# pr0g/ToyMeshPathTracer

Measured on AMD Instinct MI355X. Metric: MRays/s on sponza.obj 1920x1080 64spp at 1/2/4/8 GPUs; %HBM roofline, higher is better.
Workload: dtype f32

## Files before the change

### toymeshpathtracer_amd/csrc/tmpt_api.cpp

```cpp
#include <dlfcn.h>
#include <hip/hip_runtime.h>
#include <rccl/rccl.h>
#include <string.h>

#include <algorithm>
#include <new>
#include <chrono>
#include <string>
#include <thread>
#include <vector>

#include "tmpt.h"
#include "tmpt_internal.h"
#include "tmpt_traverse.h"
#include "tmpt_render.h"

namespace tmpt {

static thread_local std::string g_last_error;
void set_error(const std::string& msg) { g_last_error = msg; }
const char* last_error() { return g_last_error.c_str(); }

int load_obj(const char* path, std::vector<float>& tris, f3& bmin, f3& bmax);
void camera_init(tmpt_camera* cam, f3 lookFrom, f3 lookAt, f3 vup, float vfov, float aspect,
// ... 69 lines not shown
    {"builder", true, 0, 1, &Options::builder, nullptr, nullptr},
    {"layout", true, 0, 1, &Options::layout, nullptr, nullptr},
    {"leaf_max", true, 1, kLeafMaxTris, &Options::leaf_max, nullptr, nullptr},
    {"collapse", true, 0, 1, &Options::collapse, nullptr, nullptr},
    {"ploc_radius", true, 1, 256, &Options::ploc_radius, nullptr, nullptr},
    {"sah_c_leaf", true, 0, 1e6, nullptr, &Options::sah_c_leaf, nullptr},
    {"sah_c_tri", true, 0, 1e6, nullptr, &Options::sah_c_tri, nullptr},
    {"sample_block", false, 0, 1024, &Options::sample_block, nullptr, nullptr},
    {"sample_tail", false, -1, 64, &Options::sample_tail, nullptr, nullptr},
    {"sbuf_max", false, 0, 1e18, nullptr, nullptr, &Options::sbuf_max},
    {"sbuf_pair", false, 0, 1, &Options::sbuf_pair, nullptr, nullptr},
    {"pilot", false, -1, 512, &Options::pilot, nullptr, nullptr},
    {"help", false, -1, 1, &Options::help, nullptr, nullptr},
    {"pair", false, -1, 63, &Options::pair, nullptr, nullptr},
    {"balance", false, 0, 1, &Options::balance, nullptr, nullptr},
    {"dprio", false, 0, 1, &Options::dprio, nullptr, nullptr},
    {"wave_cap", false, 0, 64, &Options::wave_cap, nullptr, nullptr},
    {"pixel_chains", false, -1, 1024, &Options::pixel_chains, nullptr, nullptr},
    {"tie_defer", false, -1, 1, &Options::tie_defer, nullptr, nullptr},
    {"redo_cap", false, 0, 1 << 30, &Options::redo_cap, nullptr, nullptr},
    {"redo_inline", false, 0, 1, &Options::redo_inline, nullptr, nullptr},
    {"redo_lanes", false, 1, 64, &Options::redo_lanes, nullptr, nullptr},
    {"path_waves", false, 0, 5, &Options::path_waves, nullptr, nullptr},
    {"rowspec", false, 0, 1, &Options::rowspec, nullptr, nullptr},
    {"rowspec_wmax", false, 0, 16384, &Options::rowspec_wmax, nullptr, nullptr},
    {"rowspec_windows", false, 0, 32, &Options::rowspec_windows, nullptr, nullptr},
    {"rowspec_spread", false, -1, 100, nullptr, &Options::rowspec_spread, nullptr},
    {"rowspec_groups", false, 1, kRowSpecMaxGroups, &Options::rowspec_groups, nullptr, nullptr},
    {"rowspec_noshadow", false, 0, 1, &Options::rowspec_noshadow, nullptr, nullptr},
    {"rowspec_chase", false, 0, 1, &Options::rowspec_chase, nullptr, nullptr},
    {"rowspec_stream", false, 0, 1, &Options::rowspec_stream, nullptr, nullptr},
    {"rowstream_dynamic", false, 0, 1, &Options::rowstream_dynamic, nullptr, nullptr},
    {"row_flag_leaves", false, 0, 1, &Options::row_flag_leaves, nullptr, nullptr},
    {"row_occ", false, 0, 5, &Options::row_occ, nullptr, nullptr},
    {"wf_bins", false, 1, 8, &Options::wf_bins, nullptr, nullptr},
    {"rowstream_test_abort", false, 0, 1, &Options::rowstream_test_abort, nullptr, nullptr},
    {"tie_rule", false, 0, 1, &Options::tie_rule, nullptr, nullptr},
    {"aov_group", false, 0, 16, &Options::aov_group, nullptr, nullptr},
};

const OptionDef* find_option(const char* key)
{
    for (const OptionDef& d : kOptions)
        if (strcmp(d.name, key) == 0) return &d;
    return nullptr;
}
// ... 812 lines not shown
```

### toymeshpathtracer_amd/csrc/tmpt_internal.h

```cpp
#pragma once

#include <hip/hip_runtime.h>
#include <stdint.h>

#include <string>
#include <vector>

#include "tmpt_math.h"

namespace tmpt {

struct alignas(16) Bvh4Node {
    float4 a;
    uint4 b;
    uint4 c;
    int4 d;
};
static_assert(sizeof(Bvh4Node) == 64, "BVH4Q node is one half cache line");

constexpr int kLeafCountShift = 27;
constexpr uint32_t kLeafFirstMask = (1u << kLeafCountShift) - 1u;
constexpr int kLeafMaxTris = 16;
constexpr int kTopNodes = 120;
constexpr int kTopNodes5 = 80;
// ... 45 lines not shown
};

void build_octree(const float* tris9, int32_t n, const float bmin[3], const float bmax[3], OctreeHost& out);
uint64_t octree_digest(const OctreeHost& t);
void octree_grid(const OctreeHost& t, const float bmin[3], const float bmax[3], OctGrid& g);
int32_t octree_flat_triangles(const float* tris9, int32_t n, const OctGrid& g, std::vector<uint8_t>& flat);

struct SoaScene {
    const uint4* __restrict__ na = nullptr;
    const uint4* __restrict__ nb = nullptr;
    const uint2* __restrict__ nc = nullptr;
    const int4* __restrict__ nd = nullptr;
    const float4* __restrict__ ta = nullptr;
    const float4* __restrict__ tb = nullptr;
    const float2* __restrict__ tc = nullptr;
};

constexpr float kBoxPadRel = 1e-5f;
constexpr float kTfarSlack = 1.00001f;

constexpr int kStackTotal = 128;

constexpr int kRowSpecMaxGroups = 8;
constexpr int kRenderCounters = 32;
constexpr int kTieCounter = 24;
constexpr int kCrackCounter = 30;
constexpr int kRedoRaysCounter = 31;
constexpr int kRedoCounter = 26;

struct Options {
    int builder = 0;
    int layout = 0;
    int leaf_max = 2;
    int collapse = 0;
    int ploc_radius = 32;
    float sah_c_leaf = 0.7f, sah_c_tri = 0.5f;
    int sample_block = 0;
    int rowstream_dynamic = 1;
    int row_flag_leaves = 1;
    int row_occ = 0;
    int sample_tail = -1;
    double sbuf_max = 0.0;
    int sbuf_pair = 1;
    int pilot = -1;
    int help = -1;
    int pair = -1;
    int balance = 1;
    int dprio = 1;
    int wave_cap = 0;
    int pixel_chains = -1;
    int rowspec = 1;
    int rowspec_wmax = 0;
    int rowspec_windows = 0;
    float rowspec_spread = -1.0f;
    int rowspec_groups = 2;
    int rowspec_noshadow = 1;
    int rowspec_chase = 1;
    int rowspec_stream = 1;
    int rowstream_test_abort = 0;
    int wf_bins = 1;
    int tie_rule = 0;
    int tie_defer = -1;
    int redo_cap = 0;
    int redo_lanes = 4;
    int path_waves = 0;
    int redo_inline = 1;
    int aov_group = 0;
};
int options_parse(Options& o, const char* text, bool allow_build);
int options_set(Options& o, const char* key, double value, bool allow_build);
int options_get(const Options& o, const char* key, double* value);

struct Scene {
    int device = 0;
    int32_t n = 0;
    int32_t n_nodes = 0;
    int32_t max_depth = 0;
    Bvh4Node* nodes4 = nullptr;
    int32_t n_nodes4 = 0, depth4 = 0, leaf_max = 0, ploc_iters = 0;
    TriPre* tri_pre = nullptr;
    TriOrig* tri_orig = nullptr;
    void* soa_buf = nullptr;
    SoaScene soa;
    std::vector<float> tris_host;
    OctNode* oct = nullptr;
    int32_t* oct_refs = nullptr;
    OctView* oct_view = nullptr;
    int32_t n_oct = 0, oct_leaves = 0, oct_depth = 0;
    int32_t oct_flat = 0;
// ... 85 lines not shown
```

### toymeshpathtracer_amd/csrc/tmpt_render.hip

```cpp
#include <hip/hip_runtime.h>

#include <stdio.h>
#include <stdlib.h>
#include <string.h>

#include <algorithm>
#include <chrono>
#include <cmath>
#include <vector>

#include "tmpt_render.h"

namespace tmpt {

__device__ __forceinline__ uint64_t wballot(bool p) { return __builtin_amdgcn_ballot_w64(p); }
__device__ __forceinline__ bool wany(bool p) { return __builtin_amdgcn_ballot_w64(p) != 0; }

__device__ __forceinline__ uint64_t stamp()
{
    uint64_t t;
    __builtin_amdgcn_sched_barrier(0);
    asm volatile("s_memtime %0\n\ts_waitcnt lgkmcnt(0)" : "=s"(t)::"memory");
    __builtin_amdgcn_sched_barrier(0);
    return t;
// ... 725 lines not shown
    const uint32_t* __restrict__ dprio_cost;
    uint32_t lane_cap;
    uint32_t chunk;
    uint32_t nblk, blk;
    uint32_t blk0;
    uint32_t ua;
    float4* __restrict__ sbuf;
    uint32_t sb_ss, sb_sp;
    uint32_t pair;
    const uint32_t* __restrict__ upix;
    const uint32_t* __restrict__ ustate;
    float4* __restrict__ rs_out;
    uint32_t* __restrict__ rs_end;
    const uint32_t* __restrict__ p_dev;
    int rs_noshadow;
    const uint32_t* __restrict__ uslot;
    RsStream rss;
    uint2* __restrict__ redo;
    float4* __restrict__ redo_state;
    uint32_t redo_cap;
    uint32_t redo_inline;
    uint32_t redo_lanes;
    uint32_t oct_shadow;
};

constexpr uint32_t kSimdKeys = 8u * 8u * 2u * 16u * 4u;

__device__ __forceinline__ uint2 simd_rank(uint32_t* reg)
{
    uint32_t r = 0, d = 0;
    if (lane_id() == 0) {
        const uint32_t hw = (uint32_t)__builtin_amdgcn_s_getreg((31 << 11) | 4);
        const uint32_t xcc = (uint32_t)__builtin_amdgcn_s_getreg((31 << 11) | 20) & 7u;
        const uint32_t key = ((((xcc * 8u + ((hw >> 13) & 7u)) * 2u + ((hw >> 12) & 1u)) * 16u +
                               ((hw >> 8) & 15u)) * 4u) + ((hw >> 4) & 3u);
        r = hw & 15u;
        if (atomicAdd(&reg[2 * key], 1u) == 0) {
            d = atomicAdd(&reg[2 * kSimdKeys], 1u);
            __hip_atomic_store(&reg[2 * key + 1], d + 1u, __ATOMIC_RELAXED, __HIP_MEMORY_SCOPE_AGENT);
        } else {
            uint32_t v;
            while ((v = __hip_atomic_load(&reg[2 * key + 1], __ATOMIC_RELAXED, __HIP_MEMORY_SCOPE_AGENT)) == 0u)
                __builtin_amdgcn_s_sleep(2);
            d = v - 1u;
        }
    }
// ... 211 lines not shown
                atomicAdd(&counters[21], 1ull);
            }
        } else if (lane_id() == 0) {
            atomicAdd(&counters[20 + (rd.x >= pc.wps ? 2 : 3)], 1ull);
        }
        if (res >= res_end)
            for (int k = 0; k < 6; ++k) __builtin_amdgcn_s_sleep(127);
    }
#ifdef TMPT_EXP_WAVETIME
    const int wt_id = (int)(gtid >> 6);
    if (lane_id() == 0 && wt_id < kWaveTimeMax) g_wavetime[3 * wt_id] = __builtin_amdgcn_s_memrealtime();
#endif
    bool has_pix = false, in_query = false, qany = false;
    bool helper = false, waiting = false;
    uint32_t hown = 0;
    uint32_t pix = 0, rng = 0, smp = 0, depth = 0;
    uint32_t pf0 = 0, pf1 = 0, pf2 = 0, pf3 = 0, pf_smp = 0xFFFFFFFFu, pf_pix = 0;
    uint32_t cur_unit = 0, re0 = 0, rs0 = 0, ndraw = 0;
    bool single = false;
    uint32_t psteps = 0;
    uint64_t rs_nr = 0, rs_nl = 0, rs_lr = 0, rs_ll = 0, rs_sr = 0, rs_sl = 0, rs_st = 0;
    uint64_t pt_shade = 0, pt_node = 0, pt_leaf = 0, pt_t = PROF ? stamp() : 0;
    uint64_t ps_fetch = 0, ps_shade = 0, ps_cam = 0, ps_start = 0;
    f3 col = mk(0.0f, 0.0f, 0.0f);
    TravRay r;
    TravState ts;
    trav_init(ts, kMaxT);

    for (;;) {
        const bool wants = has_pix ? !in_query : (HELP && helper ? !in_query : !exhausted);
        const uint64_t need = wballot(wants);
        const uint64_t trav = wballot(in_query);
        int shade_min = SHADE_MIN;
        if (TAIL > 0) {
            const int act = __popcll(wballot(has_pix));
            shade_min = max(1, min(SHADE_MIN, act / TAIL));
        }
        if (need != 0 && (__popcll(need) >= shade_min || trav == 0)) {
            if (COUNT || PROF >= 3) {
                ++rs_sr;
                rs_sl += (uint64_t)__popcll(need);
                rs_st += (uint64_t)__popcll(trav);
            }
            bool cam = false, start = false, sany = false;
            f3 so = mk(0.0f, 0.0f, 0.0f), sd = so;
            const uint64_t nopix = wballot(!has_pix && !(HELP && helper) && !exhausted);
// ... 375 lines not shown
                    camera_sample(a.cam, (uint32_t)x, y, a.invW, a.invH, rng, so, sd, ndraw);
                } else {
                    camera_sample(a.cam, (uint32_t)x, y, a.invW, a.invH, rng, so, sd);
                }
                start = true;
            }
            if (PROF >= 2) {
                const uint64_t t = stamp();
                ps_cam += t - ps_t;
                ps_t = t;
            }
            if (start) {
                r = make_trav_ray(so, sd);
                trav_init(ts, kMaxT);
                qany = sany;
                if (sany) ++rays_s; else ++rays_e;
                in_query = sv.n > 0 && !ray_has_nan(so, sd);
                if (!DEFER && a.root_check && cam && in_query && !octree_root_hit(sv, so, sd, kMinT, kMaxT)) {
                    in_query = false;
                    atomicAdd(&sv.oct->ties[1], 1ull);
                }
            }
            if (PROF >= 2) ps_start += stamp() - ps_t;
        }
        if (dp0 > 0.0f) {
            float rem = 0.0f;
            if (has_pix)
                rem = smp > (uint32_t)a.smp_begin
                          ? (float)psteps * (float)((uint32_t)a.smp_end - smp) *
                                __builtin_amdgcn_rcpf((float)(smp - (uint32_t)a.smp_begin))
                          : 3.0e38f;
            for (int o = 32; o > 0; o >>= 1) rem = fmaxf(rem, __shfl_xor(rem, o));
            if (rem >= dp0) __builtin_amdgcn_s_setprio(3);
            else if (rem >= dp1) __builtin_amdgcn_s_setprio(2);
            else if (rem >= dp2) __builtin_amdgcn_s_setprio(1);
            else __builtin_amdgcn_s_setprio(0);
        }
        if (PROF) {
            const uint64_t t = stamp();
            pt_shade += t - pt_t;
            pt_t = t;
        }
        if (!wany(in_query)) {
            if (exhausted && !wany(has_pix)) break;
            if (SAMP == 4 && !wany(has_pix)) {
                const uint32_t tick = rss_ld32(&pc.rss.ctl[2]);
// ... 2 lines not shown
                    wd_tick = tick;
                    wd_time = now;
                } else if (now - wd_time > (uint64_t)pc.rss.watchdog) {
                    if (lane_id() == 0) atomicExch(&pc.rss.ctl[1], 1u);
                    exhausted = true;
                }
                __builtin_amdgcn_s_sleep(32);
            }
            continue;
        }
        for (int k = 0; k < STEPS; ++k) {
            const uint64_t q = wballot(in_query);
            const uint64_t at_leaf = q & wballot(ts.node < 0);
            const uint64_t at_node = q & ~at_leaf;
            if (q == 0) break;
            const uint32_t n_leaf = (uint32_t)__builtin_popcount((uint32_t)at_leaf) +
                                    (uint32_t)__builtin_popcount((uint32_t)(at_leaf >> 32));
            const uint32_t n_node = (uint32_t)__builtin_popcount((uint32_t)at_node) +
                                    (uint32_t)__builtin_popcount((uint32_t)(at_node >> 32));
            const bool leaf_round = n_leaf > n_node;
            if (COUNT || PROF >= 3) {
                if (!leaf_round) { ++rs_nr; rs_nl += (uint64_t)__popcll(at_node); }
                if (leaf_round) { ++rs_lr; rs_ll += (uint64_t)__popcll(at_leaf); }
            }
            if (!COUNT) {
                const bool stepping = in_query && ((ts.node < 0) == leaf_round);
                bool done = false;
                if (leaf_round) {
                    if (stepping) done = trav_step4q2_mixed<false, BLOCK, SL, true, 2, SOA, false, FLAG>(sv, r, qany, ts, st, cnt);
                } else {
                    if (stepping) done = trav_step4q2_mixed<false, BLOCK, SL, true, 1, SOA, false, FLAG>(sv, r, qany, ts, st, cnt);
                }
                if (done) in_query = false;
                if (stepping && ((kFull && pc.cost_out) || dp0 > 0.0f)) ++psteps;
            } else if (in_query && (ts.node < 0) == leaf_round) {
                TravCount c1;
                if (trav_step4q2_mixed<COUNT, BLOCK, SL, true, 0, SOA, false, FLAG>(sv, r, qany, ts, st, c1)) in_query = false;
                TravCount& dst = qany ? cnt_s : cnt;
                dst.nodes += c1.nodes;
                dst.tris += c1.tris;
                if ((kFull && pc.cost_out) || dp0 > 0.0f) ++psteps;
            }
            if (PROF) {
                const uint64_t t = stamp();
                (leaf_round ? pt_leaf : pt_node) += t - pt_t;
                pt_t = t;
            }
        }
    }
#ifdef TMPT_EXP_WAVETIME
    if (lane_id() == 0 && wt_id < kWaveTimeMax) g_wavetime[3 * wt_id + 1] = __builtin_amdgcn_s_memrealtime();
#endif
    if (DEFER && pc.redo_inline) {
        constexpr uint64_t kRedoGuard = 2000000;
        const unsigned long long waves = (unsigned long long)gridDim.x * (BLOCK / 64);
        uint32_t t = 0;
        if (lane_id() == 0) {
            atomicAdd(&counters[kRedoWaves], 1ull);
            t = (uint32_t)atomicAdd(&counters[kRedoTaken], (unsigned long long)pc.redo_lanes);
        }
        t = lane_id() < pc.redo_lanes ? (uint32_t)__shfl((int)t, 0) + lane_id() : 0xFFFFFFFFu;
        unsigned long long seen = ~0ull;
        uint64_t since = 0;
        for (;;) {
            const unsigned long long listed =
                __hip_atomic_load(&counters[kRedoCounter], __ATOMIC_RELAXED, __HIP_MEMORY_SCOPE_AGENT);
            const uint32_t lim = (uint32_t)min(listed, (unsigned long long)pc.redo_cap);
            uint2 e = make_uint2(kRedoEmpty, 0u);
// ... 46 lines not shown
            atomicAdd(&counters[2], (unsigned long long)nt);
            atomicAdd(&counters[4], (unsigned long long)nvs);
            atomicAdd(&counters[5], (unsigned long long)nts);
        }
        if (COUNT || PROF >= 3) {
            atomicAdd(&counters[6], (unsigned long long)rs_nr);
            atomicAdd(&counters[7], (unsigned long long)rs_nl);
            atomicAdd(&counters[8], (unsigned long long)rs_lr);
            atomicAdd(&counters[9], (unsigned long long)rs_ll);
            atomicAdd(&counters[10], (unsigned long long)rs_sr);
            atomicAdd(&counters[11], (unsigned long long)rs_sl);
            atomicAdd(&counters[12], (unsigned long long)rs_st);
        }
        if (PROF) {
            atomicAdd(&counters[13], (unsigned long long)pt_shade);
            atomicAdd(&counters[14], (unsigned long long)pt_node);
            atomicAdd(&counters[15], (unsigned long long)pt_leaf);
        }
        if (PROF >= 2) {
            atomicAdd(&counters[16], (unsigned long long)ps_fetch);
            atomicAdd(&counters[17], (unsigned long long)ps_shade);
            atomicAdd(&counters[18], (unsigned long long)ps_cam);
            atomicAdd(&counters[19], (unsigned long long)ps_start);
        }
    }
}

__global__ void __launch_bounds__(256) k_pair_order(const uint32_t* __restrict__ order, int64_t P, int32_t h,
                                                     uint32_t* __restrict__ paired)
{
    const int64_t r = (int64_t)blockIdx.x * 256 + threadIdx.x;
    if (r >= P) return;
    const int64_t full = P / 64, c = r / 64, i = r - c * 64;
    const int64_t m = c < full ? 64 : P - full * 64;
    const int64_t hc = c < full ? h : (m * h + 63) / 64;
    const int64_t src = i < hc ? c * h + i : P - 1 - (c * (64 - h) + (i - hc));
    paired[r] = order[src];
}

__global__ void __launch_bounds__(256) k_order_keys(const uint32_t* __restrict__ cost, int32_t W,
                                                     int32_t rows, uint32_t* __restrict__ keys,
                                                     uint32_t* __restrict__ vals)
{
    const int64_t i = (int64_t)blockIdx.x * 256 + threadIdx.x;
    if (i >= (int64_t)W * rows) return;
    const int y = (int)(i / W), x = (int)(i - (int64_t)y * W);
// ... 631 lines not shown
struct PixelChains {
    const uint32_t* cpix;
    const float4* cinit;
    int n, smp0, cspp;
};
int render_rowspec(Scene& s, const RenderArgs& a, uint32_t* d_out, unsigned long long* d_counters,
                   const PixelChains* ch = nullptr);

__global__ void __launch_bounds__(256) k_resolve_chains(PixelChains ch, const float4* __restrict__ sbuf, int32_t spp,
                                                        float spp_recip, uint32_t* __restrict__ out)
{
    const int r = blockIdx.x * 256 + threadIdx.x;
    if (r >= ch.n) return;
    const uint32_t p = ch.cpix[r];
    const float4 c0 = ch.cinit[p];
    f3 col = mk(c0.x, c0.y, c0.z);
    for (int32_t k = ch.smp0; k < spp; ++k) {
        const float4 c = sbuf[(size_t)p * (size_t)spp + (size_t)k];
        col = col + mk(c.x, c.y, c.z);
    }
    out[p] = pack_pixel(col, spp_recip);
}

static uint32_t oct_shadow_check(const Scene& s)
{
    if (!s.oct_view || s.opt.tie_rule != 0) return 0u;
    if (s.oct_flat > 0) return 1u;
    const f3 ld = light_dir();
    const float l[3] = {fabsf(ld.x), fabsf(ld.y), fabsf(ld.z)};
    for (int k = 0; k < 3; ++k)
        if (l[k] * fminf(kMinT, s.oct_grid.reach) <= s.oct_grid.drift[k]) return 1u;
    return 0u;
}

int render_persistent(Scene& s, const RenderArgs& a, uint32_t* d_out, bool count,
                      unsigned long long* d_counters)
{
    const Options& o = s.opt;
    if (!s.path_ev[0])
        for (auto& e : s.path_ev) TMPT_HIP(hipEventCreate(&e));
    constexpr int kPathSL = 16, kPathSteps = TMPT_PATH_STEPS, kShadeMin = TMPT_SHADE_MIN, kSparse = TMPT_SPARSE;
    constexpr int kPixSteps = TMPT_PIX_STEPS;
    using PathFn = decltype(&k_path<false, kBlk, kPathSL, kPathSteps, kShadeMin, 4, kSparse>);
    const bool soa = s.soa.na != nullptr;
    PathFn fn = a.jt ? (count ? (soa ? k_path<true, kBlk, kPathSL, kPathSteps, kShadeMin, 4, kSparse, 0, 0, 1, true>
                                     : k_path<true, kBlk, kPathSL, kPathSteps, kShadeMin, 4, kSparse, 0, 0, 1>)
// ... 91 lines not shown
    if (help)
        fn = waves5p ? k_path<false, kBlk, kPathSL5, kPixSteps, kShadeMin, 5, kSparse, 0, 1>
                     : k_path<false, kBlk, kPathSL, kPixSteps, kShadeMin, 4, kSparse, 0, 1>;
    else if (waves5p)
        fn = k_path<false, kBlk, kPathSL5, kPixSteps, kShadeMin, 5, kSparse>;
    if (!a.jt && !count && !prof && s.oct_view && o.tie_rule == 0)
        fn = help ? (waves5p ? k_path<false, kBlk, kPathSL5, kPixSteps, kShadeMin, 5, kSparse, 0, 1, 0, false, 2>
                             : k_path<false, kBlk, kPathSL, kPixSteps, kShadeMin, 4, kSparse, 0, 1, 0, false, 2>)
                  : (waves5p ? k_path<false, kBlk, kPathSL5, kPixSteps, kShadeMin, 5, kSparse, 0, 0, 0, false, 2>
                             : k_path<false, kBlk, kPathSL, kPixSteps, kShadeMin, 4, kSparse, 0, 0, 0, false, 2>);
    const size_t ovf_words = std::max((size_t)grid4 * (kStackTotal - kPathSL),
                                      (size_t)std::max(grid4, grid5) * (kStackTotal - kPathSL5)) * kBlk;
    const size_t head_words = (size_t)kSeg * kCtr;
    const size_t hist_words = ordered ? radix_sort_hist_words((int32_t)P) : 0;
    const size_t reg_words = ordered ? 2 * (size_t)kSimdKeys + 64 + (size_t)P : 0;
    const size_t extra_words = ordered ? (size_t)P * (4 + 5) + hist_words + reg_words : 0;
    if (ensure_ws(s, (ovf_words + head_words + extra_words) * 4)) return -1;
    uint32_t* heads = (uint32_t*)s.ws + ovf_words;
    TMPT_HIP(hipMemsetAsync(heads, 0, head_words * 4, s.stream));
    PathCtl pc;
    memset(&pc, 0, sizeof(pc));
    pc.heads = heads;
    pc.oct_shadow = oct_shadow;
    pc.P = P;
    pc.nblk = nblk;
    pc.blk = blk;
    pc.blk0 = blk0;
    pc.ua = ua;
    RenderArgs as = a;
    if (a.jt) {
        as.bmask = nblk > 1 ? blk - 1u : 2047u;
        if (nblk > 1 || pass) {
            const size_t need = sizeof(float4) * (size_t)a.spp * (size_t)a.slots;
            if (s.sbuf_bytes < need) {
                if (s.sbuf) (void)hipFree(s.sbuf);
                s.sbuf = nullptr;
                s.sbuf_bytes = 0;
                TMPT_HIP(hipMalloc(&s.sbuf, need));
                s.sbuf_bytes = need;
            }
            pc.sbuf = s.sbuf;
        }
    }
    pc.sb_ss = 1u;
    pc.sb_sp = (uint32_t)a.spp;
    pc.pair = pc.sbuf && blk >= 2u && a.spp % 2 == 0 && o.sbuf_pair ? 1u : 0u;
    {
        const int64_t waves = std::max<int64_t>(1, (int64_t)grid * (kBlk / 64));
        int64_t c = P <= waves * 16 ? 32 : 64;
        if (o.wave_cap > 0) c = o.wave_cap;
        pc.lane_cap = (uint32_t)std::max<int64_t>(1, std::min<int64_t>(64, c));
    }
    pc.chunk = std::min<uint32_t>(kChunk, pc.lane_cap);
    pc.nchunks = (uint32_t)((P + pc.chunk - 1) / pc.chunk);
    auto final_launch = [&](const RenderArgs& af) -> int {
        TMPT_HIP(hipEventRecord(s.path_ev[2], s.stream));
        fn<<<grid, kBlk, 0, s.stream>>>(view(s), af, pc, d_out, (uint32_t*)s.ws, d_counters);
        TMPT_HIP(hipGetLastError());
        TMPT_HIP(hipEventRecord(s.path_ev[3], s.stream));
        return 0;
    };
    if (!ordered) {
        const bool defer = a.jt && !count && !prof && !soa && pc.sbuf && a.root_check == 0 && o.tie_defer != 0 &&
                           !oct_shadow &&
                           (o.tie_defer > 0 || a.slots * (int64_t)a.spp >= (waves5 ? 48 : 192) * lanes);
        bool redo = defer && s.oct_view && o.tie_rule == 0;
        if (redo && o.redo_cap > 0 && s.redo_cap != (uint32_t)o.redo_cap) free_redo(s);
        if (redo && s.redo_cap == 0) {
            int64_t cap = std::min<int64_t>(1ll << 31, std::max<int64_t>(1 << 16, a.slots * (int64_t)a.spp / 128));
            if (o.redo_cap > 0) cap = o.redo_cap;
            (void)alloc_redo(s, cap);
        }
        const bool redo_nomem = redo && s.redo_cap == 0;
        if (redo_nomem) redo = false;
        PathFn fn_main = fn;
        if (redo)
            fn_main = waves5 ? k_path<false, kBlk, kPathSL5, kPathSteps, kShadeMin, 5, kSparse, 0, 0, 1, false, 1>
                             : k_path<false, kBlk, kPathSL, kPathSteps, kShadeMin, 4, kSparse, 0, 0, 1, false, 1>;
        else if (fn == fn_default && a.jt && !count && !soa && s.oct_view && o.tie_rule == 0)
            fn_main = waves5 ? k_path<false, kBlk, kPathSL5, kPathSteps, kShadeMin, 5, kSparse, 0, 0, 1, false, 2>
// ... 39 lines not shown
                TMPT_HIP(hipMemsetAsync(heads, 0, head_words * 4, s.stream));
                continue;
            }
            s.redo_late = (int64_t)(std::min<unsigned long long>(n, s.redo_cap) - std::min(traced, n));
            if (traced < std::min<unsigned long long>(n, s.redo_cap)) {
                TMPT_HIP(hipEventRecord(s.path_ev[0], s.stream));
                k_redo<kBlk, kPathSL><<<grid, kBlk, 0, s.stream>>>(view(s), as, s.redo, s.redo_cap, s.redo_state,
                                                                  pc.sbuf, pc.sb_ss, pc.sb_sp, (uint32_t*)s.ws,
                                                                  d_counters);
                TMPT_HIP(hipGetLastError());
                TMPT_HIP(hipEventRecord(s.path_ev[1], s.stream));
                s.redo_launches = 1;
            }
            break;
        }
        if (pc.sbuf) {
            k_resolve_px<<<(unsigned)((a.slots + 63) / 64), 64, 0, s.stream>>>(
                pc.sbuf, a.slots, a.spp, a.out_recip, d_out, a.smp_begin, a.smp_end, pass ? a.prog : nullptr);
            TMPT_HIP(hipGetLastError());
        }
        return 0;
    }
    s.tie_path = s.oct_view && o.tie_rule == 0 ? 1 : 0;
    uint32_t* base = heads + head_words;
    float4* state = reinterpret_cast<float4*>(base);
    uint32_t* cost = base + 4 * (size_t)P;
    uint32_t* keys = cost + P;
    uint32_t* vals = keys + P;
    uint32_t* tkeys = vals + P;
    uint32_t* tvals = tkeys + P;
    uint32_t* hist = tvals + P;
    uint32_t* simd_reg = hist + hist_words;
    RenderArgs a1 = a;
    a1.smp_end = pilot;
    a1.out_recip = 1.0f / (float)pilot;
    a1.prog = state;
    pc.cost_out = cost;
    TMPT_HIP(hipEventRecord(s.path_ev[0], s.stream));
    fn<<<grid, kBlk, 0, s.stream>>>(view(s), a1, pc, d_out, (uint32_t*)s.ws, d_counters);
    TMPT_HIP(hipGetLastError());
    TMPT_HIP(hipEventRecord(s.path_ev[1], s.stream));
    k_order_keys<<<(unsigned)((P + 255) / 256), 256, 0, s.stream>>>(cost, a.W, a.tile_rows, keys, vals);
    const int which = radix_sort_pairs(keys, vals, tkeys, tvals, (int32_t)P, 16, hist, s.stream);
    TMPT_HIP(hipMemsetAsync(heads, 0, head_words * 4, s.stream));
    RenderArgs a2 = a;
    a2.smp_begin = pilot;
    a2.prog = state;
    pc.cost_out = nullptr;
    pc.order = which ? tvals : vals;
    int64_t nch = 0;
    {
        int per1024 = 0;
        if (o.pixel_chains >= 0) per1024 = o.pixel_chains;
        nch = std::min<int64_t>(P, (P * per1024 + 1023) / 1024);
    }
    if (nch > 0) {
        const PixelChains ch{pc.order, state, (int)nch, pilot, a.spp - pilot};
        const int rc = render_rowspec(s, a, d_out, d_counters, &ch);
        if (rc < 0) return rc;
        if (rc == 0) {
            pc.order += nch;
            pc.P = P - nch;
            pc.nchunks = (uint32_t)((pc.P + pc.chunk - 1) / pc.chunk);
        }
        s.chain_pixels = rc == 0 ? nch : 0;
    }
    if (pair > 0 && pair < 64 && pc.chunk == 64u) {
        uint32_t* paired = which ? vals : tvals;
        k_pair_order<<<(unsigned)((pc.P + 255) / 256), 256, 0, s.stream>>>(pc.order, pc.P, pair, paired);
        pc.order = paired;
    }
    if (o.balance) {
        int dev_cus = 0;
        if (hipDeviceGetAttribute(&dev_cus, hipDeviceAttributeMultiprocessorCount, s.device) != hipSuccess ||
            dev_cus < 1)
            dev_cus = 256;
        const uint32_t per_cu = (uint32_t)std::max(1, grid / dev_cus);
        pc.simd_reg = simd_reg;
        pc.nsimd = (uint32_t)dev_cus * 4u;
        pc.wps = per_cu * (uint32_t)(kBlk / 64) / 4u;
        pc.claim = simd_reg + 2 * (size_t)kSimdKeys + 64;
        TMPT_HIP(hipMemsetAsync(simd_reg, 0, reg_words * 4, s.stream));
    }
    if (ordered && o.dprio && P <= 12 * lanes) {
        pc.dprio[0] = 0.32f;
        pc.dprio[1] = 0.21f;
        pc.dprio[2] = 0.105f;
        pc.dprio_cost = cost;
    }
    if (final_launch(a2)) return -1;
    s.path_launches = 2;
    return 0;
}

int render_rowstream(Scene& s, const RenderArgs& a, uint32_t* d_out, unsigned long long* d_counters)
{
    const Options& o = s.opt;
    constexpr int kPathSL = 16, kPathSteps = TMPT_ROW_STEPS, kShadeMin = TMPT_ROW_SHADE_MIN, kSparse = 2;
    const bool flag = s.oct_view && o.tie_rule == 0 && o.row_flag_leaves;
    using RsFn = decltype(&k_path<false, kBlk, kPathSL, kPathSteps, kShadeMin, 4, kSparse, 0, 0, 2>);
    const bool w5 = o.path_waves != 4;
    const RsFn fn2 = flag ? (w5 ? k_path<false, kBlk, kPathSL5, kPathSteps, kShadeMin, 5, kSparse, 0, 0, 2, false, 2>
                                : k_path<false, kBlk, kPathSL, kPathSteps, kShadeMin, 4, kSparse, 0, 0, 2, false, 2>)
                          : (w5 ? k_path<false, kBlk, kPathSL5, kPathSteps, kShadeMin, 5, kSparse, 0, 0, 2>
                                : k_path<false, kBlk, kPathSL, kPathSteps, kShadeMin, 4, kSparse, 0, 0, 2>);
    RsFn fn4 = flag ? k_path<false, kBlk, kPathSL, kPathSteps, kShadeMin, kRsOcc3, kSparse, 0, 0, 4, false, 2>
                    : k_path<false, kBlk, kPathSL, kPathSteps, kShadeMin, kRsOcc3, kSparse, 0, 0, 4>;
    const RsFn fn4_occ4 = flag ? k_path<false, kBlk, kPathSL, kPathSteps, kShadeMin, 4, kSparse, 0, 0, 4, false, 2>
                               : k_path<false, kBlk, kPathSL, kPathSteps, kShadeMin, 4, kSparse, 0, 0, 4>;
    const int rows = a.tile_rows;
    const uint32_t W = (uint32_t)a.W, spp = (uint32_t)a.spp, T = (uint32_t)kRssT;
    const size_t lcap = (size_t)a.slots * spp;
    uint32_t R = 1024;
// ... 115 lines not shown
                                        : (float)std::min(0.25, std::max(0.0, 0.055 * room - 0.015));
    S.room_lanes = (float)((double)lanes / E_est);
    S.dyn = o.rowstream_dynamic ? ((o.rowspec_windows > 0 ? 0u : 1u) | (o.rowspec_spread >= 0.0f ? 0u : 2u)) : 0u;
    TMPT_HIP(hipMemsetAsync(s.rss_buf, 0, zero_bytes, s.stream));
    {
        const size_t n = (size_t)rows * na;
        k_rss_anchors<<<(unsigned)((n + 255) / 256), 256, 0, s.stream>>>(a, S, s.rss_tab + 256 * 1024,
                                                                        s.rss_tab + 288 * 1024);
        TMPT_HIP(hipGetLastError());
    }
    RenderArgs as = a;
    as.jt = nullptr;
    as.bmask = 0u;
    as.smp_begin = 0;
    as.smp_end = a.spp;
    PathCtl pc;
    memset(&pc, 0, sizeof(pc));
    pc.heads = heads;
    pc.nblk = pc.blk = 1u;
    pc.lane_cap = 64u;
    pc.chunk = kChunk;
    pc.rs_noshadow = 1;
    pc.oct_shadow = oct_shadow_check(s);
    pc.rss = S;
    fn4<<<grid, kBlk, 0, s.stream>>>(view(s), as, pc, d_out, ovf, spec_ctr);
    TMPT_HIP(hipGetLastError());
    TMPT_HIP(hipMemcpyAsync(s.rss_host, S.ctl, 16 * sizeof(uint32_t), hipMemcpyDeviceToHost, s.stream));
    TMPT_HIP(hipStreamSynchronize(s.stream));
#ifdef TMPT_EXP_WAVETIME
    {
        std::vector<unsigned long long> w(3 * kWaveTimeMax, 0ull), r(kWaveTimeMax, 0ull), cl(kWaveTimeMax, 0ull);
        if (hipMemcpyFromSymbol(w.data(), HIP_SYMBOL(g_wavetime), w.size() * 8) == hipSuccess &&
            hipMemcpyFromSymbol(r.data(), HIP_SYMBOL(g_rowtime), r.size() * 8) == hipSuccess &&
            hipMemcpyFromSymbol(cl.data(), HIP_SYMBOL(g_claimtime), cl.size() * 8) == hipSuccess) {
            unsigned long long t0 = ~0ull, tend = 0;
            for (int i = 0; i < kWaveTimeMax; ++i)
                if (w[3 * i] && w[3 * i + 2]) {
                    t0 = std::min(t0, w[3 * i]);
                    tend = std::max(tend, w[3 * i + 2]);
                }
            std::vector<double> rt;
            for (int i = 0; i < std::min(rows, kWaveTimeMax); ++i)
                if (r[i]) rt.push_back((r[i] - t0) * 0.01);
            std::sort(rt.begin(), rt.end());
            auto q = [&](double f) { return rt.empty() ? 0.0 : rt[std::min(rt.size() - 1, (size_t)(f * (rt.size() - 1)))]; };
            fprintf(stderr, "rowstream rows %zu done at us p0/p10/p50/p90/p99/p100 %.0f/%.0f/%.0f/%.0f/%.0f/%.0f; "
// ... 208 lines not shown
        }
        q.rs.win = w;
        w += kRsMaxWin * R;
        q.rs.ws = w;
        w += kRsMaxWin * R;
        q.rs.offs = w;
        w += R + 1;
        q.rs.total = w;
        w += 1;
        q.ovf = w;
        q.heads = w + ovf_words;
        memset(&q.pc, 0, sizeof(q.pc));
        q.pc.heads = q.heads;
        q.pc.nblk = q.pc.blk = 1u;
        q.pc.lane_cap = 64u;
        q.pc.chunk = chunk;
        q.pc.upix = q.upix;
        q.pc.ustate = q.ustate;
        q.pc.rs_out = q.rs_out;
        q.pc.rs_end = q.rs_end;
        q.pc.p_dev = q.rs.total;
        q.pc.rs_noshadow = noshadow ? 1 : 0;
        q.pc.oct_shadow = oct_shadow_check(s);
        q.rs.lpix = lpix;
        q.rs.lstate = lstate;
        q.rs.lslot = lslot;
        q.rs.lcount = lcount;
        q.rs.scratch = scratch ? scratch + (size_t)q.rs.row0 * scap : nullptr;
        q.rs.scap = scap;
        q.rs.planned = spec_ctr + 8;
        q.rs.cpix = ch ? ch->cpix + q.rs.row0 : nullptr;
        q.rs.cinit = ch ? ch->cinit : nullptr;
        q.rs.cw = ch ? 1 : a.W;
        q.rs.cspp = cspp;
        q.rs.smp0 = ch ? ch->smp0 : 0;
    }
    TMPT_HIP(hipMemsetAsync(spec_ctr, 0, 24 * sizeof(unsigned long long), s.stream));
    if (noshadow) TMPT_HIP(hipMemsetAsync(lcount, 0, 4, s.stream));
    TMPT_HIP(hipEventRecord(s.rs_event[kRowSpecMaxGroups], s.stream));
    for (Group& q : gs) {
        TMPT_HIP(hipStreamWaitEvent(q.st, s.rs_event[kRowSpecMaxGroups], 0));
        k_rs_init<<<(unsigned)((q.rs.nrows + 255) / 256), 256, 0, q.st>>>(a, q.rs);
    }
    TMPT_HIP(hipGetLastError());
    const bool chase_lds = noshadow && o.rowspec_chase != 0 && (uint64_t)nwin * (uint64_t)cspp <= kChaseList;
    int it = 0;
// ... 385 lines not shown
        s.iterations = 1;
#ifdef TMPT_DIAG
        if (c[13] + c[14] + c[15]) {
            const double tot = (double)(c[13] + c[14] + c[15]);
            fprintf(stderr, "k_path wave time: shading %.1f%%, node rounds %.1f%%, leaf rounds %.1f%% "
                            "(%.3g wave-cycles)\n",
                    100.0 * c[13] / tot, 100.0 * c[14] / tot, 100.0 * c[15] / tot, tot);
            if (c[6] && c[8] && c[10])
                fprintf(stderr, "  cycles per round: node %.0f (%.1f lanes), leaf %.0f (%.1f lanes), shading %.0f "
                                "(%.1f lanes shading, %.1f traversing); rounds node %llu leaf %llu shading %llu\n",
                        (double)c[14] / c[6], (double)c[7] / c[6], (double)c[15] / c[8], (double)c[9] / c[8],
                        (double)c[13] / c[10], (double)c[11] / c[10], (double)c[12] / c[10], c[6], c[8], c[10]);
            if (c[16] + c[17] + c[18] + c[19])
                fprintf(stderr, "  shading split: ballots+pixel fetch %.1f%%, shade/finish %.1f%%, camera %.1f%%, "
                                "query set-up %.1f%% (of all wave time)\n",
                        100.0 * c[16] / tot, 100.0 * c[17] / tot, 100.0 * c[18] / tot, 100.0 * c[19] / tot);
        }
        if (count && getenv("TMPT_ROUND_LOG"))
            fprintf(stderr,
                    "k_path rounds: node %llu (%.1f lanes), leaf %llu (%.1f lanes), shade %llu "
                    "(%.1f wanting, %.1f traversing)\n",
                    c[6], c[6] ? (double)c[7] / c[6] : 0.0, c[8], c[8] ? (double)c[9] / c[8] : 0.0,
                    c[10], c[10] ? (double)c[11] / c[10] : 0.0, c[10] ? (double)c[12] / c[10] : 0.0);
#endif
    } else if (rowspec) {
        s.extend_ms = ms;
        s.extend_rays = c[3];
        s.shadow_rays = c[0] - c[3];
        s.extend_launches = s.path_launches;
        s.iterations = s.path_launches;
    } else if (!wave) {
        s.extend_ms = ms;
        s.extend_rays = c[0];
        s.node_visits = c[1];
        s.tri_tests = c[2];
        s.extend_launches = 1;
    }
    if (ray_count) *ray_count = wave ? (s.extend_rays + s.shadow_rays) : c[0];
    return 0;
}

}
```

### toymeshpathtracer_amd/csrc/tmpt_traverse.h

```cpp
#pragma once

#include "tmpt_internal.h"

namespace tmpt {

__device__ __forceinline__ float safe_inv(float d)
{
    float a = fabsf(d) < 1e-20f ? copysignf(1e-20f, d) : d;
    return __builtin_amdgcn_rcpf(a);
}

struct TravRay {
    f3 o, d;
    float ix, iy, iz;
    float ox, oy, oz;
    uint32_t offx, offy, offz;
};

__device__ __forceinline__ TravRay make_trav_ray(f3 o, f3 d)
{
    TravRay r;
    r.o = o;
    r.d = d;
    r.ix = safe_inv(d.x);
// ... 94 lines not shown
#endif

struct TravCount {
    uint32_t nodes = 0, tris = 0;
};

struct TravState {
    int node;
    int sp;
    int best;
    float bt, bu, bv;
};

__device__ __forceinline__ void trav_init(TravState& ts, float tmax)
{
    ts.node = 0;
    ts.sp = 0;
    ts.best = -1;
    ts.bt = tmax;
    ts.bu = ts.bv = 0.0f;
}

template <bool COUNT, int BLOCK, int SL, bool TOPC = false, int KIND = 0, bool SOA = false, bool NEG = false,
          bool FLAG = false>
__device__ __forceinline__ bool trav_step4q2_mixed(const SceneView& sv, const TravRay& r, bool any,
                                                   TravState& ts, TravStack<BLOCK, SL>& st,
                                                   TravCount& cnt, float tlo = 0.0f, float tmin = kMinT,
                                                   float tmax = kMaxT)
{
    if (KIND == 1 || (KIND == 0 && ts.node >= 0)) {
        if (TMPT_CHK(sv.chk, (uint32_t)ts.node < (uint32_t)sv.n_nodes4, kChkNode, ts.node)) return true;
        uint4 A, B, C;
        int4 L;
        if (SOA && (!TOPC || (uint32_t)ts.node >= st.ntop)) {
            const uint32_t k = (uint32_t)ts.node;
            A = sv.soa.na[k], B = sv.soa.nb[k], L = sv.soa.nd[k];
            const uint2 c2 = sv.soa.nc[k];
            C = make_uint4(c2.x, c2.y, 0u, 0u);
        } else if (!TOPC || (uint32_t)ts.node >= st.ntop) {
            const uint4* p = reinterpret_cast<const uint4*>(reinterpret_cast<const char*>(sv.nodes4) +
                                                            ((uint32_t)ts.node << 6));
            A = p[0], B = p[1], C = p[2];
            L = reinterpret_cast<const int4*>(p)[3];
        } else {
            const lds_u4* q = st.top + ((uint32_t)ts.node << 2);
            const u32x4 a4 = q[0], b4 = q[1], c4 = q[2], l4 = q[3];
            A = make_uint4(a4.x, a4.y, a4.z, a4.w);
            B = make_uint4(b4.x, b4.y, b4.z, b4.w);
            C = make_uint4(c4.x, c4.y, c4.z, c4.w);
            L = make_int4((int)l4.x, (int)l4.y, (int)l4.z, (int)l4.w);
        }
        if (COUNT) ++cnt.nodes;
        const float sx = exp_mul(r.ix, A.w, 0), sy = exp_mul(r.iy, A.w, 8), sz = exp_mul(r.iz, A.w, 16);
        const float bx = __builtin_fmaf(__uint_as_float(A.x), r.ix, -r.ox);
        const float by = __builtin_fmaf(__uint_as_float(A.y), r.iy, -r.oy);
        const float bz = __builtin_fmaf(__uint_as_float(A.z), r.iz, -r.oz);
        const bool ngx = r.offx != 0u, ngy = r.offy != 32u, ngz = r.offz != 64u;
        const uint32_t qnx = ngx ? B.y : B.x, qfx = ngx ? B.x : B.y;
        const uint32_t qny = ngy ? B.w : B.z, qfy = ngy ? B.z : B.w;
        const uint32_t qnz = ngz ? C.y : C.x, qfz = ngz ? C.x : C.y;
        const v2f s2x = {sx, sx}, s2y = {sy, sy}, s2z = {sz, sz};
        const v2f b2x = {bx, bx}, b2y = {by, by}, b2z = {bz, bz};
// ... 351 lines not shown
```

Baseline: 10220.

## Add top-level LDS walk rounds before mixed traversal and size path grid by occupancy

Adds a bounded pre-loop in the path kernel that advances only the lanes currently sitting on LDS-cached top BVH nodes, via a TOPONLY specialization of the node step that skips the global-memory load branches. The aim is to clear the cheap shared-memory top levels in dedicated rounds so that later voted node rounds are not a mix of LDS lanes and slow global-memory lanes. The default cap depends on the seeding mode (four steps for sample and row seeding, none for pixel seeding). It also launches the path kernel with an occupancy-derived grid, checks that the stack spill area is large enough for it, and adds counters and profiling for top-level behaviour. The trade-off is extra ballots and possibly divergent rounds where only a few lanes are active.

```diff
diff --git a/toymeshpathtracer_amd/csrc/tmpt_api.cpp b/toymeshpathtracer_amd/csrc/tmpt_api.cpp
--- a/toymeshpathtracer_amd/csrc/tmpt_api.cpp
+++ b/toymeshpathtracer_amd/csrc/tmpt_api.cpp
@@ -115,6 +115,7 @@
     {"redo_inline", false, 0, 1, &Options::redo_inline, nullptr, nullptr},
     {"redo_lanes", false, 1, 64, &Options::redo_lanes, nullptr, nullptr},
     {"path_waves", false, 0, 5, &Options::path_waves, nullptr, nullptr},
+    {"top_walk", false, -1, 8, &Options::top_walk, nullptr, nullptr},
     {"rowspec", false, 0, 1, &Options::rowspec, nullptr, nullptr},
     {"rowspec_wmax", false, 0, 16384, &Options::rowspec_wmax, nullptr, nullptr},
     {"rowspec_windows", false, 0, 32, &Options::rowspec_windows, nullptr, nullptr},
diff --git a/toymeshpathtracer_amd/csrc/tmpt_internal.h b/toymeshpathtracer_amd/csrc/tmpt_internal.h
--- a/toymeshpathtracer_amd/csrc/tmpt_internal.h
+++ b/toymeshpathtracer_amd/csrc/tmpt_internal.h
@@ -91,7 +91,8 @@
 constexpr int kStackTotal = 128;
 
 constexpr int kRowSpecMaxGroups = 8;
-constexpr int kRenderCounters = 32;
+constexpr int kRenderCounters = 48;
+constexpr int kTopCounter = 32;
 constexpr int kTieCounter = 24;
 constexpr int kCrackCounter = 30;
 constexpr int kRedoRaysCounter = 31;
@@ -134,6 +135,7 @@
     int redo_lanes = 4;
     int path_waves = 0;
     int redo_inline = 1;
+    int top_walk = -1;
     int aov_group = 0;
 };
 int options_parse(Options& o, const char* text, bool allow_build);
diff --git a/toymeshpathtracer_amd/csrc/tmpt_render.hip b/toymeshpathtracer_amd/csrc/tmpt_render.hip
--- a/toymeshpathtracer_amd/csrc/tmpt_render.hip
+++ b/toymeshpathtracer_amd/csrc/tmpt_render.hip
@@ -771,6 +771,7 @@
     uint32_t redo_inline;
     uint32_t redo_lanes;
     uint32_t oct_shadow;
+    uint32_t top_walk;
 };
 
 constexpr uint32_t kSimdKeys = 8u * 8u * 2u * 16u * 4u;
@@ -1028,6 +1029,9 @@
     uint64_t rs_nr = 0, rs_nl = 0, rs_lr = 0, rs_ll = 0, rs_sr = 0, rs_sl = 0, rs_st = 0;
     uint64_t pt_shade = 0, pt_node = 0, pt_leaf = 0, pt_t = PROF ? stamp() : 0;
     uint64_t ps_fetch = 0, ps_shade = 0, ps_cam = 0, ps_start = 0;
+    uint64_t tv_n = 0, tv_lead = 0, tv_mix = 0, tv_only = 0, tw_r = 0, tw_l = 0;
+    uint64_t pt_top = 0, pt_node_g = 0, pn_g = 0, pn_all = 0;
+    bool lead = false;
     f3 col = mk(0.0f, 0.0f, 0.0f);
     TravRay r;
     TravState ts;
@@ -1449,6 +1453,45 @@
                 }
             }
             if (PROF >= 2) ps_start += stamp() - ps_t;
+            if (COUNT && start) lead = true;
+            if (pc.top_walk) {
+                uint64_t tw_t = 0;
+                if (PROF) {
+                    tw_t = stamp();
+                    pt_shade += tw_t - pt_t;
+                }
+                for (uint32_t k = 0; k < pc.top_walk; ++k) {
+                    const bool top = in_query && ts.node >= 0 && (uint32_t)ts.node < st.ntop;
+                    const uint64_t tm = wballot(top);
+                    if (tm == 0) break;
+                    if (COUNT || PROF) {
+                        ++tw_r;
+                        tw_l += (uint64_t)__popcll(tm);
+                    }
+                    if (COUNT) {
+                        tv_n += (uint64_t)__popcll(tm);
+                        tv_lead += (uint64_t)__popcll(wballot(top && lead));
+                    }
+                    if (top) {
+                        bool done;
+                        if (!COUNT) {
+                            done = trav_step4q2_mixed<false, BLOCK, SL, true, 1, SOA, false, FLAG, true>(sv, r, qany, ts, st,
+                                                                                                        cnt);
+                        } else {
+                            TravCount c1;
+                            done = trav_step4q2_mixed<COUNT, BLOCK, SL, true, 1, SOA, false, FLAG, true>(sv, r, qany, ts, st,
+                                                                                                        c1);
+                            (qany ? cnt_s : cnt).nodes += c1.nodes;
+                        }
+                        if (done) in_query = false;
+                        if ((kFull && pc.cost_out) || dp0 > 0.0f) ++psteps;
+                    }
+                }
+                if (PROF) {
+                    pt_t = stamp();
+                    pt_top += pt_t - tw_t;
+                }
+            }
         }
         if (dp0 > 0.0f) {
             float rem = 0.0f;
@@ -1497,6 +1540,14 @@
             if (COUNT || PROF >= 3) {
                 if (!leaf_round) { ++rs_nr; rs_nl += (uint64_t)__popcll(at_node); }
                 if (leaf_round) { ++rs_lr; rs_ll += (uint64_t)__popcll(at_leaf); }
+            }
+            uint64_t top_m = 0;
+            if ((COUNT || PROF) && !leaf_round) top_m = at_node & wballot(ts.node >= 0 && (uint32_t)ts.node < st.ntop);
+            if (COUNT) {
+                tv_n += (uint64_t)__popcll(top_m);
+                tv_lead += (uint64_t)__popcll(top_m & wballot(lead));
+                if (top_m != 0) ++((at_node & ~top_m) != 0 ? tv_mix : tv_only);
+                if (in_query && (ts.node < 0) == leaf_round && !((top_m >> lane_id()) & 1ull)) lead = false;
             }
             if (!COUNT) {
                 const bool stepping = in_query && ((ts.node < 0) == leaf_round);
@@ -1519,6 +1570,13 @@
             if (PROF) {
                 const uint64_t t = stamp();
                 (leaf_round ? pt_leaf : pt_node) += t - pt_t;
+                if (!leaf_round) {
+                    ++pn_all;
+                    if ((at_node & ~top_m) != 0) {
+                        ++pn_g;
+                        pt_node_g += t - pt_t;
+                    }
+                }
                 pt_t = t;
             }
         }
@@ -1611,6 +1669,22 @@
             atomicAdd(&counters[17], (unsigned long long)ps_shade);
             atomicAdd(&counters[18], (unsigned long long)ps_cam);
             atomicAdd(&counters[19], (unsigned long long)ps_start);
+        }
+        if (COUNT) {
+            atomicAdd(&counters[kTopCounter], (unsigned long long)tv_n);
+            atomicAdd(&counters[kTopCounter + 1], (unsigned long long)tv_lead);
+            atomicAdd(&counters[kTopCounter + 2], (unsigned long long)tv_mix);
+            atomicAdd(&counters[kTopCounter + 3], (unsigned long long)tv_only);
+        }
+        if (COUNT || PROF) {
+            atomicAdd(&counters[kTopCounter + 4], (unsigned long long)tw_r);
+            atomicAdd(&counters[kTopCounter + 5], (unsigned long long)tw_l);
+        }
+        if (PROF) {
+            atomicAdd(&counters[kTopCounter + 6], (unsigned long long)pt_top);
+            atomicAdd(&counters[kTopCounter + 7], (unsigned long long)pt_node_g);
+            atomicAdd(&counters[kTopCounter + 8], (unsigned long long)pn_g);
+            atomicAdd(&counters[kTopCounter + 9], (unsigned long long)pn_all);
         }
     }
 }
@@ -2288,6 +2362,13 @@
     out[p] = pack_pixel(col, spp_recip);
 }
 
+constexpr int kTopWalkSample = 4, kTopWalkPixel = 0, kTopWalkRow = 4;
+static uint32_t top_walk_cap(const Options& o, int seeding)
+{
+    if (o.top_walk >= 0) return (uint32_t)o.top_walk;
+    return (uint32_t)(seeding == 0 ? kTopWalkSample : seeding == 1 ? kTopWalkPixel : kTopWalkRow);
+}
+
 static uint32_t oct_shadow_check(const Scene& s)
 {
     if (!s.oct_view || s.opt.tie_rule != 0) return 0u;
@@ -2425,6 +2506,7 @@
     memset(&pc, 0, sizeof(pc));
     pc.heads = heads;
     pc.oct_shadow = oct_shadow;
+    pc.top_walk = top_walk_cap(o, a.jt ? 0 : 1);
     pc.P = P;
     pc.nblk = nblk;
     pc.blk = blk;
@@ -2456,9 +2538,9 @@
     }
     pc.chunk = std::min<uint32_t>(kChunk, pc.lane_cap);
     pc.nchunks = (uint32_t)((P + pc.chunk - 1) / pc.chunk);
-    auto final_launch = [&](const RenderArgs& af) -> int {
+    auto final_launch = [&](const RenderArgs& af, int grid_final) -> int {
         TMPT_HIP(hipEventRecord(s.path_ev[2], s.stream));
-        fn<<<grid, kBlk, 0, s.stream>>>(view(s), af, pc, d_out, (uint32_t*)s.ws, d_counters);
+        fn<<<grid_final, kBlk, 0, s.stream>>>(view(s), af, pc, d_out, (uint32_t*)s.ws, d_counters);
         TMPT_HIP(hipGetLastError());
         TMPT_HIP(hipEventRecord(s.path_ev[3], s.stream));
         return 0;
@@ -2544,6 +2626,11 @@
         return 0;
     }
     s.tie_path = s.oct_view && o.tie_rule == 0 ? 1 : 0;
+    const int grid_px = occupancy_grid((const void*)fn, kBlk, 0, s.device);
+    if ((size_t)grid_px * kBlk * (kStackTotal - (waves5p ? kPathSL5 : kPathSL)) > ovf_words) {
+        set_error("tmpt_render: internal: stack spill area sized for fewer lanes");
+        return -1;
+    }
     uint32_t* base = heads + head_words;
     float4* state = reinterpret_cast<float4*>(base);
     uint32_t* cost = base + 4 * (size_t)P;
@@ -2559,7 +2646,7 @@
     a1.prog = state;
     pc.cost_out = cost;
     TMPT_HIP(hipEventRecord(s.path_ev[0], s.stream));
-    fn<<<grid, kBlk, 0, s.stream>>>(view(s), a1, pc, d_out, (uint32_t*)s.ws, d_counters);
+    fn<<<grid_px, kBlk, 0, s.stream>>>(view(s), a1, pc, d_out, (uint32_t*)s.ws, d_counters);
     TMPT_HIP(hipGetLastError());
     TMPT_HIP(hipEventRecord(s.path_ev[1], s.stream));
     k_order_keys<<<(unsigned)((P + 255) / 256), 256, 0, s.stream>>>(cost, a.W, a.tile_rows, keys, vals);
@@ -2597,7 +2684,7 @@
         if (hipDeviceGetAttribute(&dev_cus, hipDeviceAttributeMultiprocessorCount, s.device) != hipSuccess ||
             dev_cus < 1)
             dev_cus = 256;
-        const uint32_t per_cu = (uint32_t)std::max(1, grid / dev_cus);
+        const uint32_t per_cu = (uint32_t)std::max(1, grid_px / dev_cus);
         pc.simd_reg = simd_reg;
         pc.nsimd = (uint32_t)dev_cus * 4u;
         pc.wps = per_cu * (uint32_t)(kBlk / 64) / 4u;
@@ -2610,7 +2697,7 @@
         pc.dprio[2] = 0.105f;
         pc.dprio_cost = cost;
     }
-    if (final_launch(a2)) return -1;
+    if (final_launch(a2, grid_px)) return -1;
     s.path_launches = 2;
     return 0;
 }
@@ -2772,6 +2859,7 @@
     pc.chunk = kChunk;
     pc.rs_noshadow = 1;
     pc.oct_shadow = oct_shadow_check(s);
+    pc.top_walk = top_walk_cap(o, 2);
     pc.rss = S;
     fn4<<<grid, kBlk, 0, s.stream>>>(view(s), as, pc, d_out, ovf, spec_ctr);
     TMPT_HIP(hipGetLastError());
@@ -3026,6 +3114,7 @@
         q.pc.p_dev = q.rs.total;
         q.pc.rs_noshadow = noshadow ? 1 : 0;
         q.pc.oct_shadow = oct_shadow_check(s);
+        q.pc.top_walk = top_walk_cap(o, 2);
         q.rs.lpix = lpix;
         q.rs.lstate = lstate;
         q.rs.lslot = lslot;
@@ -3457,6 +3546,26 @@
                     "(%.1f wanting, %.1f traversing)\n",
                     c[6], c[6] ? (double)c[7] / c[6] : 0.0, c[8], c[8] ? (double)c[9] / c[8] : 0.0,
                     c[10], c[10] ? (double)c[11] / c[10] : 0.0, c[10] ? (double)c[12] / c[10] : 0.0);
+        {
+            const unsigned long long* t = c + kTopCounter;
+            const unsigned long long nv = c[1] + c[4];
+            if (count && getenv("TMPT_ROUND_LOG") && nv)
+                fprintf(stderr,
+                        "k_path top levels: %.4f of node lane-steps on an LDS node, %.4f of those before the query's "
+                        "first other step (%.2f per query); voted node rounds with LDS lanes %.4f, of them mixed "
+                        "with global lanes %.4f; top-walk rounds %llu (%.1f lanes)\n",
+                        (double)t[0] / nv, t[0] ? (double)t[1] / t[0] : 0.0, (double)t[1] / (double)c[0],
+                        c[6] ? (double)(t[2] + t[3]) / c[6] : 0.0, t[2] + t[3] ? (double)t[2] / (t[2] + t[3]) : 0.0,
+                        t[4], t[4] ? (double)t[5] / t[4] : 0.0);
+            if (t[9])
+                fprintf(stderr,
+                        "  node rounds with a global-side lane: %llu of %llu, %.0f cycles each; without: %.0f cycles "
+                        "each; top-walk rounds %llu (%.1f lanes), %.0f cycles each, %.2f%% of wave time\n",
+                        t[8], t[9], t[8] ? (double)t[7] / t[8] : 0.0,
+                        t[9] > t[8] ? (double)(c[14] - t[7]) / (t[9] - t[8]) : 0.0, t[4],
+                        t[4] ? (double)t[5] / t[4] : 0.0, t[4] ? (double)t[6] / t[4] : 0.0,
+                        100.0 * t[6] / (double)(c[13] + c[14] + c[15] + t[6]));
+        }
 #endif
     } else if (rowspec) {
         s.extend_ms = ms;
diff --git a/toymeshpathtracer_amd/csrc/tmpt_traverse.h b/toymeshpathtracer_amd/csrc/tmpt_traverse.h
--- a/toymeshpathtracer_amd/csrc/tmpt_traverse.h
+++ b/toymeshpathtracer_amd/csrc/tmpt_traverse.h
@@ -140,7 +140,7 @@
 }
 
 template <bool COUNT, int BLOCK, int SL, bool TOPC = false, int KIND = 0, bool SOA = false, bool NEG = false,
-          bool FLAG = false>
+          bool FLAG = false, bool TOPONLY = false>
 __device__ __forceinline__ bool trav_step4q2_mixed(const SceneView& sv, const TravRay& r, bool any,
                                                    TravState& ts, TravStack<BLOCK, SL>& st,
                                                    TravCount& cnt, float tlo = 0.0f, float tmin = kMinT,
@@ -150,12 +150,12 @@
         if (TMPT_CHK(sv.chk, (uint32_t)ts.node < (uint32_t)sv.n_nodes4, kChkNode, ts.node)) return true;
         uint4 A, B, C;
         int4 L;
-        if (SOA && (!TOPC || (uint32_t)ts.node >= st.ntop)) {
+        if (!TOPONLY && SOA && (!TOPC || (uint32_t)ts.node >= st.ntop)) {
             const uint32_t k = (uint32_t)ts.node;
             A = sv.soa.na[k], B = sv.soa.nb[k], L = sv.soa.nd[k];
             const uint2 c2 = sv.soa.nc[k];
             C = make_uint4(c2.x, c2.y, 0u, 0u);
-        } else if (!TOPC || (uint32_t)ts.node >= st.ntop) {
+        } else if (!TOPONLY && (!TOPC || (uint32_t)ts.node >= st.ntop)) {
             const uint4* p = reinterpret_cast<const uint4*>(reinterpret_cast<const char*>(sv.nodes4) +
                                                             ((uint32_t)ts.node << 6));
             A = p[0], B = p[1], C = p[2];
```

Result: faster. 10400 (median of 6 runs) (+1.7%).
